# sparsemat/sprs

Measured on NVIDIA H100. Metric: csr_spmv_f64_gflops, higher is better.
Workload: dtype f64

## Files before the change

sprs_b200/csrc/common.cuh:

```cuda
#pragma once
#include <cuda_runtime.h>

#include <cstdint>
#include <cstdio>
#include <cstring>
#include <string>
#include <vector>

#include "../../include/sprs_b200.h"

constexpr int SPRS_E2E_MAX_CHUNKS = 8;
constexpr int SPRS_E2E_DEFAULT_CHUNKS = 8;

struct sprs_b200_ctx {
    int device = 0;
    int sm_count = 132;
    size_t l2_bytes = 0;
    cudaStream_t stream = nullptr;
    std::string last_error;
    uint64_t launches = 0;
    uint64_t pol_evict_first = 0, pol_evict_last = 0;
    void* h_stage = nullptr;
    size_t h_stage_bytes = 0;
    void* d_scratch[4] = {nullptr, nullptr, nullptr, nullptr};
    size_t d_scratch_bytes[4] = {0, 0, 0, 0};
    cudaStream_t side_stream = nullptr;
    cudaEvent_t ev_fork = nullptr, ev_join = nullptr;
    cudaStream_t copy_stream = nullptr;
    cudaEvent_t ev_chunk[SPRS_E2E_MAX_CHUNKS] = {};
    cudaEvent_t ev_copied = nullptr;
};

struct sprs_b200_csmat {
    sprs_b200_ctx* ctx = nullptr;
    int storage = SPRS_B200_CSR;
    uint64_t rows = 0, cols = 0, nnz = 0;
    uint64_t outer = 0, inner = 0;
    int indptr_bytes = 4;
    void* d_indptr = nullptr;
    uint32_t* d_indices = nullptr;
    double* d_data = nullptr;
    bool owns = true;
    bool pooled = false;
    uint32_t* d_tile_row = nullptr;
    void* d_tile_k = nullptr;
    double* d_carry = nullptr;
    uint64_t n_tiles = 0;
    uint32_t* d_hot_col = nullptr;
    uint32_t* d_hot_idx = nullptr;
    uint32_t n_hot = 0;
    mutable sprs_b200_csmat* csr_cache = nullptr;
    mutable std::vector<uint64_t> e2e_tiles, e2e_rows;
    mutable std::vector<uint64_t> push_tiles, push_rows;
};

#define SPRS_FAIL(ctx, code, ...)                                  \
    do {                                                           \
        char _buf[512];                                            \
        snprintf(_buf, sizeof(_buf), __VA_ARGS__);                 \
        sprs_b200_set_error((ctx), _buf);                          \
        return (code);                                             \
    } while (0)

#define SPRS_CUDA(ctx, expr)                                                              \
    do {                                                                                  \
        cudaError_t _e = (expr);                                                          \
        if (_e != cudaSuccess)                                                            \
            SPRS_FAIL((ctx), SPRS_B200_ERR_CUDA, "%s failed: %s (%s:%d)", #expr,          \
                      cudaGetErrorString(_e), __FILE__, __LINE__);                        \
    } while (0)

#define SPRS_TRY(expr)                      \
    do {                                    \
        int _s = (expr);                    \
        if (_s != SPRS_B200_OK) return _s;  \
    } while (0)

void sprs_b200_set_error(const sprs_b200_ctx* ctx, const char* msg);

static inline cudaStream_t pick_stream(sprs_b200_ctx*, void* stream) {
    return (cudaStream_t)stream;
}

int ctx_scratch(sprs_b200_ctx* ctx, int i, size_t bytes, void** out);
int ctx_stage(sprs_b200_ctx* ctx, size_t bytes, void** out);

constexpr int SPMV_MAX_TARGETS = 8;
struct SpmvTargets {
    double* p[SPMV_MAX_TARGETS];
    int n;
};

int spmv_prepare(sprs_b200_ctx* ctx, sprs_b200_csmat* m, cudaStream_t s, bool hot_set = true);
int spmv_tile_nnz();
int spmv_launch(sprs_b200_ctx* ctx, const sprs_b200_csmat* m, const double* d_x, double* d_y,
                int accumulate, cudaStream_t s);
int spmv_launch_targets(sprs_b200_ctx* ctx, const sprs_b200_csmat* m, const double* d_x,
                        const SpmvTargets& yt, int accumulate, cudaStream_t s);
int spmv_launch_tile_range(sprs_b200_ctx* ctx, const sprs_b200_csmat* m, const double* d_x,
                           double* d_y, int accumulate, uint64_t t0, uint64_t t1, cudaStream_t s);
int csmat_chunk_table(sprs_b200_ctx* ctx, const sprs_b200_csmat* m, uint64_t n_chunks, bool taper,
                      cudaStream_t s, std::vector<uint64_t>* tiles, std::vector<uint64_t>* rows);
int ctx_side_stream(sprs_b200_ctx* ctx);
// ... 24 lines not shown
```

sprs_b200/csrc/ptx.cuh:

```cuda
#pragma once
#include "common.cuh"

static __device__ __forceinline__ void fence_proxy_async() {
    asm volatile("fence.proxy.async.shared::cta;" ::: "memory");
}
static __device__ __forceinline__ uint64_t policy_evict_first() {
    uint64_t p;
    asm volatile("createpolicy.fractional.L2::evict_first.b64 %0, 1.0;" : "=l"(p));
    return p;
}
static __device__ __forceinline__ uint64_t policy_evict_last() {
    uint64_t p;
    asm volatile("createpolicy.fractional.L2::evict_last.b64 %0, 1.0;" : "=l"(p));
    return p;
}
static __device__ __forceinline__ double ldg_f64_hint(const double* p, uint64_t policy) {
    double v;
    asm("ld.global.nc.L2::cache_hint.f64 %0, [%1], %2;" : "=d"(v) : "l"(p), "l"(policy));
    return v;
}

static __device__ __forceinline__ uint32_t ldg_stream_u32(const uint32_t* p, uint64_t policy) {
    uint32_t v;
    asm("ld.global.nc.L1::no_allocate.L2::cache_hint.u32 %0, [%1], %2;"
        : "=r"(v) : "l"(p), "l"(policy));
    return v;
}
static __device__ __forceinline__ double ldg_stream_f64(const double* p, uint64_t policy) {
    double v;
    asm("ld.global.nc.L1::no_allocate.L2::cache_hint.f64 %0, [%1], %2;"
        : "=d"(v) : "l"(p), "l"(policy));
    return v;
}

static __device__ __forceinline__ void bulk_s2g(void* dst, const void* src_smem, uint32_t bytes) {
    asm volatile("cp.async.bulk.global.shared::cta.bulk_group [%0], [%1], %2;" ::"l"(dst),
                 "r"(smem_u32(src_smem)), "r"(bytes)
                 : "memory");
}
static __device__ __forceinline__ void bulk_commit_group() {
    asm volatile("cp.async.bulk.commit_group;" ::: "memory");
}
static __device__ __forceinline__ void bulk_wait_group_read0() {
    asm volatile("cp.async.bulk.wait_group.read 0;" ::: "memory");
}
static __device__ __forceinline__ void bulk_wait_group0() {
    asm volatile("cp.async.bulk.wait_group 0;" ::: "memory");
}
```

sprs_b200/csrc/spmv.cu:

```cuda

#include "common.cuh"
#include "ptx.cuh"
#include "scan.cuh"

#include <algorithm>
#include <cstdlib>

namespace {

constexpr int SPMV_STAGE_ROWS = 66;
constexpr uint32_t SPMV_ROW_COST = 16;

template <typename P>
__global__ void tile_cut_kernel(const P* __restrict__ indptr, uint32_t rows, uint64_t nnz,
                                uint64_t n_tiles, uint32_t w, uint32_t row_cost,
                                uint32_t* __restrict__ tile_row, P* __restrict__ tile_k) {
    const uint64_t t = blockIdx.x * (uint64_t)blockDim.x + threadIdx.x;
    if (t > n_tiles) return;
    if (t == n_tiles) {
        tile_row[t] = rows;
        tile_k[t] = (P)nnz;
        return;
    }
    const uint64_t d = t * (uint64_t)w;
    uint32_t lo = 0, hi = rows;
    while (lo < hi) {
        const uint32_t mid = lo + (hi - lo + 1) / 2;
        if ((uint64_t)indptr[mid] + (uint64_t)row_cost * mid <= d)
            lo = mid;
        else
            hi = mid - 1;
    }
    uint64_t k = d - (uint64_t)row_cost * lo;
    const uint64_t row_end = lo < rows ? (uint64_t)indptr[(size_t)lo + 1] : nnz;
    if (k > row_end) k = row_end;
    tile_row[t] = lo;
    tile_k[t] = (P)k;
}

struct RowSink {
    double* y;
    const SpmvTargets* yt;
    double* carry_slot;
    uint32_t r1;
    int accumulate;
    double* stage;
    uint32_t stage_off;
};
template <bool MULTI>
__device__ __forceinline__ void sink_row(const RowSink& k, uint64_t r, double sum) {
    if (r < k.r1) {
        const double v = k.accumulate ? __dadd_rn(k.y[r], sum) : sum;
        k.y[r] = v;
        if (MULTI) {
#pragma unroll
            if (k.stage) {
                k.stage[(uint32_t)r - k.stage_off] = v;
            } else {
#pragma unroll
                for (int q = 1; q < SPMV_MAX_TARGETS; ++q)
                    if (q < k.yt->n) k.yt->p[q][r] = v;
            }
        }
    } else {
        *k.carry_slot = sum;
    }
}

constexpr uint32_t HOT_TAG = 0x80000000u;
template <bool HOT>
__device__ __forceinline__ double gather_x(const double* __restrict__ x, const double* hot,
                                           uint32_t c, uint64_t polx) {
    if (HOT && (c & HOT_TAG)) return hot[c & ~HOT_TAG];
    return ldg_f64_hint(x + c, polx);
}

template <typename P, int G, int U, bool MULTI, bool HOT>
__device__ __forceinline__ void rows_direct(const RowSink& k, const P* __restrict__ indptr,
                                            const uint32_t* __restrict__ indices,
                                            const double* __restrict__ data,
                                            const double* __restrict__ x, const double* hot, P k0, P k1,
                                            uint32_t r0, uint32_t r_last, P b_first,
                                            uint64_t pol_stream, uint64_t polx, int lane) {
    constexpr int NG = 32 / G;
    constexpr unsigned FULL = 0xffffffffu;
    static_assert(G >= 4, "tiny rows have their own sweep: groups start at 4 lanes");
    const int gid = lane / G, gl = lane % G;
    P b = b_first;
    for (uint32_t rbase = r0;; rbase += 31) {
        if (rbase != r0) {
            const uint32_t rr = rbase + lane;
            b = (rr >= rbase && rr <= r_last + 1) ? indptr[rr] : (P)0;
        }
        const int nrows = (r_last - rbase + 1) < 31 ? (int)(r_last - rbase + 1) : 31;
        P ms = b, me = __shfl_down_sync(FULL, b, 1);
        ms = ms > k0 ? ms : k0;
        me = me < k1 ? me : k1;
        if (lane >= nrows || me < ms) me = ms;
        const bool tiny = lane < nrows && (me - ms) <= (P)(2 * U);
        if (__any_sync(FULL, tiny && me > ms)) {
            double acc = 0.0;
#pragma unroll
            for (int st = 0; st < 2; ++st) {
                const P q = ms + (P)(st * U);
                uint32_t c[U];
                double v[U], xv[U];
#pragma unroll
                for (int u = 0; u < U; ++u)
                    c[u] = (tiny && q + (P)u < me) ? ldg_stream_u32(indices + q + (P)u, pol_stream) : 0u;
#pragma unroll
                for (int u = 0; u < U; ++u)
                    v[u] = (tiny && q + (P)u < me) ? ldg_stream_f64(data + q + (P)u, pol_stream) : 0.0;
#pragma unroll
                for (int u = 0; u < U; ++u)
                    xv[u] = (tiny && q + (P)u < me) ? gather_x<HOT>(x, hot, c[u], polx) : 0.0;
#pragma unroll
                for (int u = 0; u < U; ++u)
                    if (tiny && q + (P)u < me) acc = __dadd_rn(acc, __dmul_rn(v[u], xv[u]));
                if (!__any_sync(FULL, tiny && q + (P)U < me)) break;
            }
            if (tiny) sink_row<MULTI>(k, (uint64_t)rbase + lane, acc);
        } else if (tiny) {
            sink_row<MULTI>(k, (uint64_t)rbase + lane, 0.0);
        }
        unsigned todo = __ballot_sync(FULL, lane < nrows && !tiny);
        while (todo) {
            int j = -1;
#pragma unroll
            for (int g = 0; g < NG; ++g) {
                if (todo) {
                    const int jj = __ffs(todo) - 1;
                    todo &= todo - 1;
                    if (gid == g) j = jj;
                }
            }
            const bool valid = j >= 0;
            const int js = valid ? j : 0;
            P s = __shfl_sync(FULL, b, js);
            P e = __shfl_sync(FULL, b, js + 1);
            s = s > k0 ? s : k0;
            e = e < k1 ? e : k1;
            if (!valid || e < s) e = s;
            const bool is_long = (G < 32) && (e - s) > (P)(4 * G * U);
            double acc = 0.0;
            for (P q = s + gl; q < (is_long ? s : e); q += (P)(G * U)) {
                uint32_t c[U];
                double v[U], xv[U];
#pragma unroll
                for (int u = 0; u < U; ++u)
                    c[u] = q + (P)(u * G) < e ? ldg_stream_u32(indices + q + (P)(u * G), pol_stream) : 0u;
#pragma unroll
                for (int u = 0; u < U; ++u)
                    v[u] = q + (P)(u * G) < e ? ldg_stream_f64(data + q + (P)(u * G), pol_stream) : 0.0;
#pragma unroll
                for (int u = 0; u < U; ++u)
                    xv[u] = q + (P)(u * G) < e ? gather_x<HOT>(x, hot, c[u], polx) : 0.0;
#pragma unroll
                for (int u = 0; u < U; ++u)
                    if (q + (P)(u * G) < e) acc = __dadd_rn(acc, __dmul_rn(v[u], xv[u]));
            }
#pragma unroll
            for (int o = G / 2; o > 0; o >>= 1) acc = __dadd_rn(acc, __shfl_xor_sync(FULL, acc, o));
            if (gl == 0 && valid && !is_long) sink_row<MULTI>(k, (uint64_t)rbase + j, acc);
            if (G < 32) {
                unsigned pending = __ballot_sync(FULL, gl == 0 && is_long);
                while (pending) {
                    const int src = __ffs(pending) - 1;
                    pending &= pending - 1;
                    const P qs = __shfl_sync(FULL, s, src), qe = __shfl_sync(FULL, e, src);
                    const int jj = __shfl_sync(FULL, j, src);
                    double a2 = 0.0;
                    for (P q = qs + lane; q < qe; q += (P)(32 * U)) {
                        uint32_t c[U];
                        double v[U], xv[U];
#pragma unroll
                        for (int u = 0; u < U; ++u)
                            c[u] = q + (P)(u * 32) < qe ? ldg_stream_u32(indices + q + (P)(u * 32), pol_stream) : 0u;
#pragma unroll
                        for (int u = 0; u < U; ++u)
                            v[u] = q + (P)(u * 32) < qe ? ldg_stream_f64(data + q + (P)(u * 32), pol_stream) : 0.0;
#pragma unroll
                        for (int u = 0; u < U; ++u)
                            xv[u] = q + (P)(u * 32) < qe ? gather_x<HOT>(x, hot, c[u], polx) : 0.0;
#pragma unroll
                        for (int u = 0; u < U; ++u)
                            if (q + (P)(u * 32) < qe) a2 = __dadd_rn(a2, __dmul_rn(v[u], xv[u]));
                    }
#pragma unroll
                    for (int o = 16; o > 0; o >>= 1) a2 = __dadd_rn(a2, __shfl_xor_sync(FULL, a2, o));
                    if (lane == 0) sink_row<MULTI>(k, (uint64_t)rbase + jj, a2);
                }
            }
        }
        if (r_last - rbase < 31) break;
    }
}

template <typename P, int NWARPS, int MINB, int U, bool MULTI, bool HOT>
__global__ void __launch_bounds__(NWARPS * 32, MINB)
    spmv_rows_kernel(const P* __restrict__ indptr, const uint32_t* __restrict__ indices,
                     const double* __restrict__ data, const uint32_t* __restrict__ tile_row,
                     const P* __restrict__ tile_k, const double* __restrict__ x,
                     const __grid_constant__ SpmvTargets yt,
                     double* __restrict__ carry, uint64_t nnz, uint32_t rows, uint32_t t_begin,
                     uint32_t t_end , int accumulate,
                     uint64_t pol_stream , uint64_t polx ,
                     int stage_rows ,
                     const uint32_t* __restrict__ hot_col ,
                     uint32_t n_hot) {
    const int lane = threadIdx.x & 31, warp = threadIdx.x >> 5;
    extern __shared__ __align__(16) double hot_x[];
    if constexpr (HOT) {
        for (uint32_t q = threadIdx.x; q < n_hot; q += NWARPS * 32)
            hot_x[q] = ldg_f64_hint(x + hot_col[q], polx);
        __syncthreads();
    }
    const uint32_t GW = gridDim.x * NWARPS;
    RowSink sink;
    sink.y = yt.p[0];
    sink.yt = &yt;
    sink.accumulate = accumulate;
    sink.stage = nullptr;
    sink.stage_off = 0;
    double* my_stage = nullptr;
    if constexpr (MULTI) {
        __shared__ __align__(16) double stage_all[NWARPS * SPMV_STAGE_ROWS];
        my_stage = stage_all + warp * SPMV_STAGE_ROWS;
    }
    const uint32_t par = MULTI ? (uint32_t)(((uintptr_t)yt.p[1] >> 3) & 1) : 0u;
    uint32_t t = t_begin + blockIdx.x * NWARPS + warp;
    if (t >= t_end) return;
    uint32_t r0 = tile_row[t], r1 = tile_row[t + 1];
    P k0 = tile_k[t], k1 = tile_k[t + 1];
    P b_first = (uint64_t)r0 + lane <= (r1 < rows ? (uint64_t)r1 + 1 : (uint64_t)r1)
                    ? indptr[(size_t)r0 + lane] : (P)0;
    for (;;) {
        const uint32_t tn = t + GW;
        uint32_t r0n = 0, r1n = 0;
        P k0n = 0, k1n = 0;
        if (tn < t_end) {
            r0n = tile_row[tn];
            r1n = tile_row[tn + 1];
            k0n = tile_k[tn];
            k1n = tile_k[tn + 1];
        }
        sink.carry_slot = carry + t;
        sink.r1 = r1;
        if (MULTI && stage_rows) {
            const uint32_t base = (r0 + par) & ~1u;
            const bool fits = r1 > r0 && (r1 + par - base) <= (uint32_t)SPMV_STAGE_ROWS;
            sink.stage = fits ? my_stage : nullptr;
            sink.stage_off = base - par;
            if (fits) {
                if (lane == 0) bulk_wait_group_read0();
                __syncwarp();
            }
        }
        const uint32_t r_last = r1 < rows ? r1 : r1 - 1;
        const uint64_t cnt = k1 - k0, nr = (uint64_t)(r_last - r0) + 1;
#define SPMV_ROWS(G)                                                                            \
    rows_direct<P, G, U, MULTI, HOT>(sink, indptr, indices, data, x, hot_x, k0, k1, r0, r_last,   \
                                     b_first, pol_stream, polx, lane)
        if (cnt <= 24 * nr)
            SPMV_ROWS(4);
        else if (cnt <= 48 * nr)
            SPMV_ROWS(8);
        else if (cnt <= 96 * nr)
            SPMV_ROWS(16);
        else
            SPMV_ROWS(32);
#undef SPMV_ROWS
        if (MULTI && sink.stage) {
            fence_proxy_async();
            __syncwarp();
            if (lane == 0) {
                uint32_t lo = r0, hi = r1;
                if ((lo + par) & 1u) {
                    const double v = my_stage[lo - sink.stage_off];
                    for (int q = 1; q < yt.n; ++q) yt.p[q][lo] = v;
                    ++lo;
                }
                if ((hi - lo) & 1u) {
                    --hi;
                    const double v = my_stage[hi - sink.stage_off];
                    for (int q = 1; q < yt.n; ++q) yt.p[q][hi] = v;
                }
                if (hi > lo) {
                    for (int q = 1; q < yt.n; ++q)
                        bulk_s2g(yt.p[q] + lo, my_stage + (lo - sink.stage_off), (hi - lo) * 8u);
                    bulk_commit_group();
                }
            }
            sink.stage = nullptr;
        }
        if (tn >= t_end) break;
        const P b_next = (uint64_t)r0n + lane <= (r1n < rows ? (uint64_t)r1n + 1 : (uint64_t)r1n)
                             ? indptr[(size_t)r0n + lane] : (P)0;
        t = tn;
        r0 = r0n;
        r1 = r1n;
        k0 = k0n;
        k1 = k1n;
        b_first = b_next;
    }
    if (MULTI && stage_rows && lane == 0) bulk_wait_group0();
}

__global__ void spmv_fixup_kernel(const uint32_t* __restrict__ tile_row,
                                  const double* __restrict__ carry, SpmvTargets yt,
                                  uint64_t n_tiles) {
    const uint64_t t = blockIdx.x * (uint64_t)blockDim.x + threadIdx.x;
    if (t + 1 >= n_tiles) return;
    const uint32_t row = tile_row[t + 1];
    if (t > 0 && tile_row[t] == row) return;
    uint64_t lo = t + 1, hi = n_tiles - 1;
    for (uint64_t step = 1; lo + step < hi; step <<= 1) {
        if (tile_row[lo + step + 1] > row) {
            hi = lo + step;
            break;
        }
        lo += step;
    }
    while (lo < hi) {
        const uint64_t mid = lo + (hi - lo) / 2;
        if (tile_row[mid + 1] > row)
            hi = mid;
        else
            lo = mid + 1;
    }
    double sum = carry[t];
#pragma unroll 8
    for (uint64_t u = t + 1; u < lo; ++u) sum = __dadd_rn(sum, carry[u]);
    const double v = __dadd_rn(yt.p[0][row], sum);
#pragma unroll
    for (int q = 0; q < SPMV_MAX_TARGETS; ++q)
        if (q < yt.n) yt.p[q][row] = v;
}

__device__ __forceinline__ void apply_carries_ending_in(const uint32_t* __restrict__ tile_row,
                                                        const double* carry, double* y,
                                                        uint64_t u) {
    const uint32_t row = tile_row[u];
    if (tile_row[u + 1] == row) return;
    uint64_t hi = u, lo = 1;
    for (uint64_t step = 1; step < hi; step <<= 1) {
        if (tile_row[hi - step] < row) {
            lo = hi - step + 1;
            break;
        }
        hi -= step;
    }
    while (lo < hi) {
        const uint64_t mid = lo + (hi - lo) / 2;
        if (tile_row[mid] >= row)
            hi = mid;
        else
            lo = mid + 1;
    }
    double sum = __ldcg(carry + lo - 1);
    for (uint64_t v = lo; v < u; ++v) sum = __dadd_rn(sum, __ldcg(carry + v));
    y[row] = __dadd_rn(__ldcg(y + row), sum);
}

__global__ void spmv_fixup_range_kernel(const uint32_t* __restrict__ tile_row, const double* carry,
                                        double* y, uint64_t u_lo, uint64_t u_hi) {
    const uint64_t u = u_lo + blockIdx.x * (uint64_t)blockDim.x + threadIdx.x;
    if (u >= 1 && u < u_hi) apply_carries_ending_in(tile_row, carry, y, u);
}

struct SpmvVariant {
    int wt, row_cost;
};
SpmvVariant spmv_variant() {
    static SpmvVariant v = [] {
        SpmvVariant d{1024, (int)SPMV_ROW_COST};
        if (const char* e = getenv("SPRS_B200_SPMV_VARIANT")) {
            int a, rc = (int)SPMV_ROW_COST;
            const int got = sscanf(e, "%d,%d", &a, &rc);
            if (got >= 1 && a >= 64 && rc >= 0) d = SpmvVariant{a, rc};
        }
        return d;
    }();
    return v;
}

constexpr int SPMV_NWARPS = 8, SPMV_CTAS_PER_SM = 5, SPMV_LOADS_IN_FLIGHT = 4;

constexpr int SPMV_HOT_NWARPS = 32, SPMV_HOT_CTAS_PER_SM = 1;
constexpr uint32_t SPMV_HOT_SLOTS = 24576;
constexpr uint32_t SPMV_HOT_MAX_SLOTS = 26624;
constexpr uint64_t SPMV_HOT_MIN_NNZ = 1ull << 25;
constexpr double SPMV_HOT_MIN_SHARE = 0.10;

struct SpmvHot {
    uint32_t k;
    bool forced;
};
SpmvHot spmv_hot() {
    static SpmvHot h = [] {
        SpmvHot d{SPMV_HOT_SLOTS, false};
        const char* e = getenv("SPRS_B200_SPMV_HOT");
        if (e && strcmp(e, "auto") != 0) {
            const long k = atol(e);
            d = SpmvHot{(uint32_t)(k < 0 ? 0 : k > (long)SPMV_HOT_MAX_SLOTS ? SPMV_HOT_MAX_SLOTS : k), true};
        }
        return d;
    }();
    return h;
}

template <typename P, bool MULTI, bool HOT>
auto* spmv_kernel() {
    constexpr int U = SPMV_LOADS_IN_FLIGHT;
    if constexpr (HOT)
        return spmv_rows_kernel<P, SPMV_HOT_NWARPS, SPMV_HOT_CTAS_PER_SM, U, MULTI, true>;
    else
        return spmv_rows_kernel<P, SPMV_NWARPS, SPMV_CTAS_PER_SM, U, MULTI, false>;
}

template <typename P>
int launch_variant(sprs_b200_ctx* ctx, const sprs_b200_csmat* m, const double* d_x,
                   const SpmvTargets& yt, int accumulate, uint64_t t0, uint64_t t1,
                   cudaStream_t s) {
    if (m->n_tiles >= 0xffffffffull)
        SPRS_FAIL(ctx, SPRS_B200_ERR_UNSUPPORTED, "spmv: more than 2^32 tiles");
    const bool multi = yt.n > 1, hot = m->n_hot > 0;
    auto kern = hot ? (multi ? spmv_kernel<P, true, true>() : spmv_kernel<P, false, true>())
                    : (multi ? spmv_kernel<P, true, false>() : spmv_kernel<P, false, false>());
    const int nwarps = hot ? SPMV_HOT_NWARPS : SPMV_NWARPS;
    const int ctas = hot ? SPMV_HOT_CTAS_PER_SM : SPMV_CTAS_PER_SM;
    static bool configured_flags[64][4] = {};
    bool& configured = configured_flags[ctx->device & 63][(multi ? 1 : 0) + (hot ? 2 : 0)];
    if (!configured) {
        int carve;
        if (hot) {
            const int dyn = (int)(spmv_hot().k * sizeof(double));
            const int per_cta = dyn + (multi ? nwarps * SPMV_STAGE_ROWS * 8 : 0) + 1024;
            SPRS_CUDA(ctx, cudaFuncSetAttribute(kern, cudaFuncAttributeMaxDynamicSharedMemorySize, dyn));
            carve = (int)((100ull * ctas * per_cta + 228 * 1024 - 1) / (228 * 1024));
        } else {
            carve = multi ? 15 : 0;
            if (const char* e = getenv("SPRS_B200_SPMV_CARVEOUT")) carve = atoi(e);
        }
        SPRS_CUDA(ctx, cudaFuncSetAttribute(kern, cudaFuncAttributePreferredSharedMemoryCarveout,
                                            carve));
        configured = true;
    }
    int stage_rows = 0;
    if (multi) {
        stage_rows = yt.n > 2 ? SPMV_STAGE_ROWS : 0;
        if (const char* e = getenv("SPRS_B200_SPMV_PEER_STORES")) {
            if (e[0] == 'd') stage_rows = 0;
            if (e[0] == 't') stage_rows = SPMV_STAGE_ROWS;
        }
        for (int q = 2; q < yt.n; ++q)
            if ((((uintptr_t)yt.p[q] ^ (uintptr_t)yt.p[1]) >> 3) & 1) stage_rows = 0;
    }
    uint64_t grid = (uint64_t)ctx->sm_count * ctas;
    const uint64_t need = (t1 - t0 + nwarps - 1) / nwarps;
    if (grid > need) grid = need;
    const size_t smem = hot ? m->n_hot * sizeof(double) : 0;
    kern<<<(unsigned)grid, nwarps * 32, smem, s>>>((const P*)m->d_indptr,
                                                   hot ? m->d_hot_idx : m->d_indices,
                                                   m->d_data, m->d_tile_row, (const P*)m->d_tile_k, d_x, yt,
                                                   m->d_carry,
                                                   m->nnz, (uint32_t)m->rows, (uint32_t)t0,
                                                   (uint32_t)t1, accumulate, ctx->pol_evict_first,
                                                   ctx->pol_evict_last, stage_rows, m->d_hot_col,
                                                   m->n_hot);
    return SPRS_B200_OK;
}

__device__ __forceinline__ void add_aggregated(uint32_t* counts, uint32_t key, unsigned active) {
    const unsigned peers = __match_any_sync(active, key);
    if ((int)(threadIdx.x & 31) == __ffs(peers) - 1) atomicAdd(counts + key, (uint32_t)__popc(peers));
}

__global__ void hot_count_kernel(const uint32_t* __restrict__ indices, uint64_t nnz,
                                 uint32_t* __restrict__ counts) {
    const uint64_t stride = (uint64_t)gridDim.x * blockDim.x;
    for (uint64_t base = blockIdx.x * (uint64_t)blockDim.x + (threadIdx.x & ~31u); base < nnz;
         base += stride) {
        const uint64_t i = base + (threadIdx.x & 31);
        const bool valid = i < nnz;
        const unsigned active = __ballot_sync(0xffffffffu, valid);
        if (valid) add_aggregated(counts, indices[i], active);
    }
}

__global__ void hot_count_hist_kernel(const uint32_t* __restrict__ counts, uint32_t cols,
                                      uint32_t hi, uint32_t* __restrict__ hist) {
    const uint64_t stride = (uint64_t)gridDim.x * blockDim.x;
    for (uint64_t base = blockIdx.x * (uint64_t)blockDim.x + (threadIdx.x & ~31u); base < cols;
         base += stride) {
        const uint64_t i = base + (threadIdx.x & 31);
        const uint32_t c = i < cols ? counts[i] : 0u;
        const bool take = c > 0 && (hi == ~0u || (c >> 16) == hi);
        const unsigned active = __ballot_sync(0xffffffffu, take);
        if (take) add_aggregated(hist, hi == ~0u ? c >> 16 : c & 0xffffu, active);
    }
}

__global__ void hot_flag_kernel(const uint32_t* __restrict__ counts, uint32_t cols, uint32_t thr,
                                const uint32_t* __restrict__ tie_rank, uint32_t ties,
                                uint8_t* __restrict__ flag) {
    const uint64_t i = blockIdx.x * (uint64_t)blockDim.x + threadIdx.x;
    if (i >= cols) return;
    const uint32_t c = counts[i];
    flag[i] = tie_rank ? (c > thr || (c == thr && tie_rank[i] < ties)) : c == thr;
}

__global__ void hot_map_kernel(uint32_t* __restrict__ counts_map, uint32_t cols,
                               const uint8_t* __restrict__ sel, const uint32_t* __restrict__ slot,
                               uint32_t* __restrict__ hot_col, unsigned long long* hot_nnz) {
    const uint64_t i = blockIdx.x * (uint64_t)blockDim.x + threadIdx.x;
    if (i >= cols) return;
    if (sel[i]) {
        const uint32_t q = slot[i];
        atomicAdd(hot_nnz, (unsigned long long)counts_map[i]);
        hot_col[q] = (uint32_t)i;
        counts_map[i] = HOT_TAG | q;
    } else {
        counts_map[i] = (uint32_t)i;
    }
}

__global__ void hot_tag_kernel(const uint32_t* __restrict__ indices, uint64_t nnz,
                               const uint32_t* __restrict__ map, uint32_t* __restrict__ tagged) {
    const uint64_t stride = (uint64_t)gridDim.x * blockDim.x;
    for (uint64_t i = blockIdx.x * (uint64_t)blockDim.x + threadIdx.x; i < nnz; i += stride)
        tagged[i] = map[indices[i]];
}

int spmv_prepare_hot(sprs_b200_ctx* ctx, sprs_b200_csmat* m, cudaStream_t s) {
    const SpmvHot cfg = spmv_hot();
    if (cfg.k == 0 || m->nnz == 0 || m->cols == 0 || m->cols >= HOT_TAG) return SPRS_B200_OK;
    if (!cfg.forced && m->nnz < SPMV_HOT_MIN_NNZ) return SPRS_B200_OK;
    const uint32_t cols = (uint32_t)m->cols;
    uint32_t *counts = nullptr, *hist = nullptr, *slot = nullptr, *hot_col = nullptr,
             *hot_idx = nullptr;
    uint8_t* flag = nullptr;
    unsigned long long* d_hot_nnz = nullptr;
    const unsigned grid_nnz =
        (unsigned)std::min<uint64_t>((m->nnz + 255) / 256, (uint64_t)ctx->sm_count * 16);
    const unsigned grid_cols = (unsigned)((cols + 255) / 256);
    auto build = [&]() -> int {
        if (cudaMalloc((void**)&counts, cols * sizeof(uint32_t)) != cudaSuccess ||
            cudaMalloc((void**)&hist, 65536 * sizeof(uint32_t)) != cudaSuccess ||
            cudaMalloc((void**)&flag, cols) != cudaSuccess ||
            cudaMalloc((void**)&slot, (cols + 1ull) * sizeof(uint32_t)) != cudaSuccess ||
            cudaMalloc((void**)&d_hot_nnz, sizeof(unsigned long long)) != cudaSuccess)
            return SPRS_B200_OK;
        SPRS_CUDA(ctx, cudaMemsetAsync(counts, 0, cols * sizeof(uint32_t), s));
        SPRS_CUDA(ctx, cudaMemsetAsync(hist, 0, 65536 * sizeof(uint32_t), s));
        SPRS_CUDA(ctx, cudaMemsetAsync(d_hot_nnz, 0, sizeof(unsigned long long), s));
        hot_count_kernel<<<grid_nnz, 256, 0, s>>>(m->d_indices, m->nnz, counts);
        hot_count_hist_kernel<<<grid_cols, 256, 0, s>>>(counts, cols, ~0u, hist);
        ctx->launches += 2;
        std::vector<uint32_t> h(65536);
        SPRS_CUDA(ctx, cudaMemcpyAsync(h.data(), hist, 65536 * sizeof(uint32_t),
                                       cudaMemcpyDeviceToHost, s));
        SPRS_CUDA(ctx, cudaStreamSynchronize(s));
        uint64_t above = 0, referenced = 0;
        for (uint32_t b = 0; b < 65536; ++b) referenced += h[b];
        uint32_t k = cfg.k, thr = 1, ties = 0xffffffffu;
        if (referenced > k) {
            uint32_t bhi = 65535;
            while (above + h[bhi] < k) above += h[bhi--];
            SPRS_CUDA(ctx, cudaMemsetAsync(hist, 0, 65536 * sizeof(uint32_t), s));
            hot_count_hist_kernel<<<grid_cols, 256, 0, s>>>(counts, cols, bhi, hist);
            ctx->launches += 1;
            SPRS_CUDA(ctx, cudaMemcpyAsync(h.data(), hist, 65536 * sizeof(uint32_t),
                                           cudaMemcpyDeviceToHost, s));
            SPRS_CUDA(ctx, cudaStreamSynchronize(s));
            uint32_t blo = 65535;
            while (above + h[blo] < k) above += h[blo--];
            thr = (bhi << 16) | blo;
            ties = k - (uint32_t)above;
        } else {
            k = (uint32_t)referenced;
        }
        hot_flag_kernel<<<grid_cols, 256, 0, s>>>(counts, cols, thr, nullptr, 0, flag);
        ctx->launches += 1;
        SPRS_TRY((device_exclusive_scan<uint8_t, uint32_t>(ctx, flag, cols, slot, s)));
        hot_flag_kernel<<<grid_cols, 256, 0, s>>>(counts, cols, thr, slot, ties, flag);
        ctx->launches += 1;
        SPRS_TRY((device_exclusive_scan<uint8_t, uint32_t>(ctx, flag, cols, slot, s)));
        if (cudaMalloc((void**)&hot_col, k * sizeof(uint32_t)) != cudaSuccess) return SPRS_B200_OK;
        hot_map_kernel<<<grid_cols, 256, 0, s>>>(counts, cols, flag, slot, hot_col, d_hot_nnz);
        ctx->launches += 1;
        unsigned long long hot_nnz = 0;
        SPRS_CUDA(ctx, cudaMemcpyAsync(&hot_nnz, d_hot_nnz, sizeof(hot_nnz), cudaMemcpyDeviceToHost, s));
        SPRS_CUDA(ctx, cudaStreamSynchronize(s));
        if (!cfg.forced && (double)hot_nnz < SPMV_HOT_MIN_SHARE * (double)m->nnz) return SPRS_B200_OK;
        if (cudaMalloc((void**)&hot_idx, m->nnz * sizeof(uint32_t) + 16) != cudaSuccess)
            return SPRS_B200_OK;
        hot_tag_kernel<<<grid_nnz, 256, 0, s>>>(m->d_indices, m->nnz, counts, hot_idx);
        ctx->launches += 1;
        SPRS_CUDA(ctx, cudaStreamSynchronize(s));
        SPRS_CUDA(ctx, cudaGetLastError());
        m->d_hot_col = hot_col;
        m->d_hot_idx = hot_idx;
        m->n_hot = k;
        return SPRS_B200_OK;
    };
    const int st = build();
    if (m->n_hot == 0) {
        cudaGetLastError();
        if (hot_col) cudaFree(hot_col);
        if (hot_idx) cudaFree(hot_idx);
    }
    if (counts) cudaFree(counts);
    if (hist) cudaFree(hist);
    if (flag) cudaFree(flag);
    if (slot) cudaFree(slot);
    if (d_hot_nnz) cudaFree(d_hot_nnz);
    return st;
}

int check_spmv_args(sprs_b200_ctx* ctx, const sprs_b200_csmat* m) {
    if (m->storage != SPRS_B200_CSR)
        SPRS_FAIL(ctx, SPRS_B200_ERR_STORAGE, "Storage mismatch: spmv needs a CSR mirror");
    if (!m->d_tile_row) SPRS_FAIL(ctx, SPRS_B200_ERR_ARGUMENT, "csmat has no SpMV partition");
    return SPRS_B200_OK;
}

}

int spmv_tile_nnz() { return spmv_variant().wt; }

int spmv_prepare(sprs_b200_ctx* ctx, sprs_b200_csmat* m, cudaStream_t s, bool hot_set) {
    if (m->storage != SPRS_B200_CSR) return SPRS_B200_OK;
    const uint32_t w = (uint32_t)spmv_tile_nnz();
    const uint32_t row_cost = (uint32_t)spmv_variant().row_cost;
    const uint64_t total = m->nnz + (uint64_t)row_cost * m->rows;
    m->n_tiles = total == 0 ? 1 : (total + w - 1) / w;
    SPRS_CUDA(ctx, cudaMalloc((void**)&m->d_tile_row, (m->n_tiles + 1) * sizeof(uint32_t)));
    SPRS_CUDA(ctx, cudaMalloc((void**)&m->d_tile_k, (m->n_tiles + 1) * (size_t)m->indptr_bytes));
    SPRS_CUDA(ctx, cudaMalloc((void**)&m->d_carry, m->n_tiles * sizeof(double)));
    const uint64_t n = m->n_tiles + 1;
    const unsigned grid = (unsigned)((n + 255) / 256);
    if (m->indptr_bytes == 4)
        tile_cut_kernel<uint32_t><<<grid, 256, 0, s>>>((const uint32_t*)m->d_indptr, (uint32_t)m->rows,
                                                       m->nnz, m->n_tiles, w, row_cost, m->d_tile_row,
                                                       (uint32_t*)m->d_tile_k);
    else
        tile_cut_kernel<uint64_t><<<grid, 256, 0, s>>>((const uint64_t*)m->d_indptr, (uint32_t)m->rows,
                                                       m->nnz, m->n_tiles, w, row_cost, m->d_tile_row,
                                                       (uint64_t*)m->d_tile_k);
    ctx->launches += 1;
    SPRS_CUDA(ctx, cudaGetLastError());
    if (hot_set) SPRS_TRY(spmv_prepare_hot(ctx, m, s));
    return SPRS_B200_OK;
}

int spmv_launch_targets(sprs_b200_ctx* ctx, const sprs_b200_csmat* m, const double* d_x,
                        const SpmvTargets& yt, int accumulate, cudaStream_t s) {
    SPRS_TRY(check_spmv_args(ctx, m));
    if (m->rows == 0) return SPRS_B200_OK;
    if (m->indptr_bytes == 4)
        SPRS_TRY(launch_variant<uint32_t>(ctx, m, d_x, yt, accumulate, 0, m->n_tiles, s));
    else
        SPRS_TRY(launch_variant<uint64_t>(ctx, m, d_x, yt, accumulate, 0, m->n_tiles, s));
    ctx->launches += 1;
    if (m->n_tiles > 1) {
        const unsigned fgrid = (unsigned)((m->n_tiles - 1 + 255) / 256);
        spmv_fixup_kernel<<<fgrid, 256, 0, s>>>(m->d_tile_row, m->d_carry, yt, m->n_tiles);
        ctx->launches += 1;
// ... 34 lines not shown
```

Measured before the change: 226.9.

## Split hot x cache across CTA pairs via clusters and distributed shared memory

Extends the shared-memory cache of frequently referenced x entries by launching the hot SpMV kernel as 2-CTA clusters. A small set of the hottest columns is duplicated in each CTA, and a larger set is split between the pair, with remote entries read through DSMEM (mapa + ld.shared::cluster). This roughly doubles effective cached x capacity to cut L2/HBM gathers, at the cost of cluster barriers at kernel start and exit, slower remote shared loads, and more preprocessing kernels and host syncs.

Result: faster. 230.7 (median of 6 runs) (+1.7%).

```diff
diff --git a/sprs_b200/csrc/common.cuh b/sprs_b200/csrc/common.cuh
--- a/sprs_b200/csrc/common.cuh
+++ b/sprs_b200/csrc/common.cuh
@@ -49,6 +49,7 @@
     uint32_t* d_hot_col = nullptr;
     uint32_t* d_hot_idx = nullptr;
     uint32_t n_hot = 0;
+    uint32_t n_hot_split = 0;
     mutable sprs_b200_csmat* csr_cache = nullptr;
     mutable std::vector<uint64_t> e2e_tiles, e2e_rows;
     mutable std::vector<uint64_t> push_tiles, push_rows;
diff --git a/sprs_b200/csrc/ptx.cuh b/sprs_b200/csrc/ptx.cuh
--- a/sprs_b200/csrc/ptx.cuh
+++ b/sprs_b200/csrc/ptx.cuh
@@ -33,6 +33,25 @@
     return v;
 }
 
+static __device__ __forceinline__ uint32_t cluster_ctarank() {
+    uint32_t r;
+    asm volatile("mov.u32 %0, %%cluster_ctarank;" : "=r"(r));
+    return r;
+}
+static __device__ __forceinline__ void cluster_arrive_release() {
+    asm volatile("barrier.cluster.arrive.release;" ::: "memory");
+}
+static __device__ __forceinline__ void cluster_wait_acquire() {
+    asm volatile("barrier.cluster.wait.acquire;" ::: "memory");
+}
+static __device__ __forceinline__ double ld_dsmem_f64(const double* p, uint32_t rank) {
+    uint32_t a;
+    double v;
+    asm volatile("mapa.shared::cluster.u32 %0, %1, %2;" : "=r"(a) : "r"(smem_u32(p)), "r"(rank));
+    asm volatile("ld.shared::cluster.f64 %0, [%1];" : "=d"(v) : "r"(a));
+    return v;
+}
+
 static __device__ __forceinline__ void bulk_s2g(void* dst, const void* src_smem, uint32_t bytes) {
     asm volatile("cp.async.bulk.global.shared::cta.bulk_group [%0], [%1], %2;" ::"l"(dst),
                  "r"(smem_u32(src_smem)), "r"(bytes)
diff --git a/sprs_b200/csrc/spmv.cu b/sprs_b200/csrc/spmv.cu
--- a/sprs_b200/csrc/spmv.cu
+++ b/sprs_b200/csrc/spmv.cu
@@ -67,21 +67,36 @@
     }
 }
 
-constexpr uint32_t HOT_TAG = 0x80000000u;
-template <bool HOT>
+constexpr uint32_t HOT_TAG = 0x80000000u, HOT_SPLIT = 0x40000000u, HOT_OWNER_SHIFT = 29,
+                   HOT_SLOT = 0x1fffffffu;
+enum { HOT_OFF = 0, HOT_CTA = 1, HOT_CLUSTER = 2 };
+#ifdef __NVCC__
+#define SPMV_HOT_CLUSTERS 1
+#else
+#define SPMV_HOT_CLUSTERS 0
+#endif
+template <int HOT>
 __device__ __forceinline__ double gather_x(const double* __restrict__ x, const double* hot,
-                                           uint32_t c, uint64_t polx) {
-    if (HOT && (c & HOT_TAG)) return hot[c & ~HOT_TAG];
+                                           uint32_t c, uint64_t polx, uint32_t rank) {
+    if (HOT != HOT_OFF && (c & HOT_TAG)) {
+        const double* p = hot + (c & HOT_SLOT);
+#if SPMV_HOT_CLUSTERS
+        if (HOT == HOT_CLUSTER && (c & HOT_SPLIT) && ((c >> HOT_OWNER_SHIFT) & 1u) != rank)
+            return ld_dsmem_f64(p, rank ^ 1u);
+#endif
+        return *p;
+    }
     return ldg_f64_hint(x + c, polx);
 }
 
-template <typename P, int G, int U, bool MULTI, bool HOT>
+template <typename P, int G, int U, bool MULTI, int HOT>
 __device__ __forceinline__ void rows_direct(const RowSink& k, const P* __restrict__ indptr,
                                             const uint32_t* __restrict__ indices,
                                             const double* __restrict__ data,
                                             const double* __restrict__ x, const double* hot, P k0, P k1,
                                             uint32_t r0, uint32_t r_last, P b_first,
-                                            uint64_t pol_stream, uint64_t polx, int lane) {
+                                            uint64_t pol_stream, uint64_t polx, int lane,
+                                            uint32_t rank) {
     constexpr int NG = 32 / G;
     constexpr unsigned FULL = 0xffffffffu;
     static_assert(G >= 4, "tiny rows have their own sweep: groups start at 4 lanes");
@@ -113,7 +128,7 @@
                     v[u] = (tiny && q + (P)u < me) ? ldg_stream_f64(data + q + (P)u, pol_stream) : 0.0;
 #pragma unroll
                 for (int u = 0; u < U; ++u)
-                    xv[u] = (tiny && q + (P)u < me) ? gather_x<HOT>(x, hot, c[u], polx) : 0.0;
+                    xv[u] = (tiny && q + (P)u < me) ? gather_x<HOT>(x, hot, c[u], polx, rank) : 0.0;
 #pragma unroll
                 for (int u = 0; u < U; ++u)
                     if (tiny && q + (P)u < me) acc = __dadd_rn(acc, __dmul_rn(v[u], xv[u]));
@@ -154,7 +169,7 @@
                     v[u] = q + (P)(u * G) < e ? ldg_stream_f64(data + q + (P)(u * G), pol_stream) : 0.0;
 #pragma unroll
                 for (int u = 0; u < U; ++u)
-                    xv[u] = q + (P)(u * G) < e ? gather_x<HOT>(x, hot, c[u], polx) : 0.0;
+                    xv[u] = q + (P)(u * G) < e ? gather_x<HOT>(x, hot, c[u], polx, rank) : 0.0;
 #pragma unroll
                 for (int u = 0; u < U; ++u)
                     if (q + (P)(u * G) < e) acc = __dadd_rn(acc, __dmul_rn(v[u], xv[u]));
@@ -181,7 +196,7 @@
                             v[u] = q + (P)(u * 32) < qe ? ldg_stream_f64(data + q + (P)(u * 32), pol_stream) : 0.0;
 #pragma unroll
                         for (int u = 0; u < U; ++u)
-                            xv[u] = q + (P)(u * 32) < qe ? gather_x<HOT>(x, hot, c[u], polx) : 0.0;
+                            xv[u] = q + (P)(u * 32) < qe ? gather_x<HOT>(x, hot, c[u], polx, rank) : 0.0;
 #pragma unroll
                         for (int u = 0; u < U; ++u)
                             if (q + (P)(u * 32) < qe) a2 = __dadd_rn(a2, __dmul_rn(v[u], xv[u]));
@@ -196,7 +211,17 @@
     }
 }
 
-template <typename P, int NWARPS, int MINB, int U, bool MULTI, bool HOT>
+template <int HOT>
+__device__ __forceinline__ void hot_cluster_exit() {
+#if SPMV_HOT_CLUSTERS
+    if constexpr (HOT == HOT_CLUSTER) {
+        cluster_arrive_release();
+        cluster_wait_acquire();
+    }
+#endif
+}
+
+template <typename P, int NWARPS, int MINB, int U, bool MULTI, int HOT>
 __global__ void __launch_bounds__(NWARPS * 32, MINB)
     spmv_rows_kernel(const P* __restrict__ indptr, const uint32_t* __restrict__ indices,
                      const double* __restrict__ data, const uint32_t* __restrict__ tile_row,
@@ -207,14 +232,25 @@
                      uint64_t pol_stream , uint64_t polx ,
                      int stage_rows ,
                      const uint32_t* __restrict__ hot_col ,
-                     uint32_t n_hot) {
+                     uint32_t n_hot, uint32_t n_dup ) {
     const int lane = threadIdx.x & 31, warp = threadIdx.x >> 5;
     extern __shared__ __align__(16) double hot_x[];
-    if constexpr (HOT) {
+    uint32_t rank = 0;
+    if constexpr (HOT == HOT_CTA) {
         for (uint32_t q = threadIdx.x; q < n_hot; q += NWARPS * 32)
             hot_x[q] = ldg_f64_hint(x + hot_col[q], polx);
         __syncthreads();
     }
+#if SPMV_HOT_CLUSTERS
+    if constexpr (HOT == HOT_CLUSTER) {
+        rank = cluster_ctarank();
+        const uint32_t n_mine = n_dup + (n_hot - n_dup + 1 - rank) / 2;
+        for (uint32_t q = threadIdx.x; q < n_mine; q += NWARPS * 32)
+            hot_x[q] = ldg_f64_hint(x + hot_col[q < n_dup ? q : n_dup + 2 * (q - n_dup) + rank], polx);
+        cluster_arrive_release();
+        cluster_wait_acquire();
+    }
+#endif
     const uint32_t GW = gridDim.x * NWARPS;
     RowSink sink;
     sink.y = yt.p[0];
@@ -229,7 +265,10 @@
     }
     const uint32_t par = MULTI ? (uint32_t)(((uintptr_t)yt.p[1] >> 3) & 1) : 0u;
     uint32_t t = t_begin + blockIdx.x * NWARPS + warp;
-    if (t >= t_end) return;
+    if (t >= t_end) {
+        hot_cluster_exit<HOT>();
+        return;
+    }
     uint32_t r0 = tile_row[t], r1 = tile_row[t + 1];
     P k0 = tile_k[t], k1 = tile_k[t + 1];
     P b_first = (uint64_t)r0 + lane <= (r1 < rows ? (uint64_t)r1 + 1 : (uint64_t)r1)
@@ -260,7 +299,7 @@
         const uint64_t cnt = k1 - k0, nr = (uint64_t)(r_last - r0) + 1;
 #define SPMV_ROWS(G)                                                                            \
     rows_direct<P, G, U, MULTI, HOT>(sink, indptr, indices, data, x, hot_x, k0, k1, r0, r_last,   \
-                                     b_first, pol_stream, polx, lane)
+                                     b_first, pol_stream, polx, lane, rank)
         if (cnt <= 24 * nr)
             SPMV_ROWS(4);
         else if (cnt <= 48 * nr)
@@ -304,6 +343,7 @@
         b_first = b_next;
     }
     if (MULTI && stage_rows && lane == 0) bulk_wait_group0();
+    hot_cluster_exit<HOT>();
 }
 
 __global__ void spmv_fixup_kernel(const uint32_t* __restrict__ tile_row,
@@ -387,35 +427,114 @@
 constexpr int SPMV_NWARPS = 8, SPMV_CTAS_PER_SM = 5, SPMV_LOADS_IN_FLIGHT = 4;
 
 constexpr int SPMV_HOT_NWARPS = 32, SPMV_HOT_CTAS_PER_SM = 1;
-constexpr uint32_t SPMV_HOT_SLOTS = 24576;
 constexpr uint32_t SPMV_HOT_MAX_SLOTS = 26624;
+constexpr uint32_t SPMV_HOT_AUTO_DUP = 4096, SPMV_HOT_AUTO_SPLIT = 16384;
 constexpr uint64_t SPMV_HOT_MIN_NNZ = 1ull << 25;
 constexpr double SPMV_HOT_MIN_SHARE = 0.10;
 
 struct SpmvHot {
-    uint32_t k;
+    uint32_t dup, split;
     bool forced;
+    uint32_t per_cta() const { return dup + split; }
 };
 SpmvHot spmv_hot() {
     static SpmvHot h = [] {
-        SpmvHot d{SPMV_HOT_SLOTS, false};
+        SpmvHot d{SPMV_HOT_AUTO_DUP, SPMV_HOT_AUTO_SPLIT, false};
         const char* e = getenv("SPRS_B200_SPMV_HOT");
         if (e && strcmp(e, "auto") != 0) {
-            const long k = atol(e);
-            d = SpmvHot{(uint32_t)(k < 0 ? 0 : k > (long)SPMV_HOT_MAX_SLOTS ? SPMV_HOT_MAX_SLOTS : k), true};
+            const char* plus = strchr(e, '+');
+            long a = atol(e), b = plus ? atol(plus + 1) : 0;
+            a = a < 0 ? 0 : a > (long)SPMV_HOT_MAX_SLOTS ? SPMV_HOT_MAX_SLOTS : a;
+            b = b < 0 ? 0 : b > (long)SPMV_HOT_MAX_SLOTS - a ? SPMV_HOT_MAX_SLOTS - a : b;
+            d = SpmvHot{(uint32_t)a, (uint32_t)b, true};
         }
         return d;
     }();
     return h;
 }
 
-template <typename P, bool MULTI, bool HOT>
-auto* spmv_kernel() {
-    constexpr int U = SPMV_LOADS_IN_FLIGHT;
-    if constexpr (HOT)
-        return spmv_rows_kernel<P, SPMV_HOT_NWARPS, SPMV_HOT_CTAS_PER_SM, U, MULTI, true>;
-    else
-        return spmv_rows_kernel<P, SPMV_NWARPS, SPMV_CTAS_PER_SM, U, MULTI, false>;
+template <typename P>
+using SpmvKernel = decltype(&spmv_rows_kernel<P, SPMV_NWARPS, SPMV_CTAS_PER_SM,
+                                              SPMV_LOADS_IN_FLIGHT, false, HOT_OFF>);
+template <typename P>
+SpmvKernel<P> spmv_kernel(bool multi, int hot) {
+    constexpr int U = SPMV_LOADS_IN_FLIGHT, HW = SPMV_HOT_NWARPS, HB = SPMV_HOT_CTAS_PER_SM;
+    switch (hot) {
+        case HOT_CTA:
+            return multi ? spmv_rows_kernel<P, HW, HB, U, true, HOT_CTA>
+                         : spmv_rows_kernel<P, HW, HB, U, false, HOT_CTA>;
+        case HOT_CLUSTER:
+            return multi ? spmv_rows_kernel<P, HW, HB, U, true, HOT_CLUSTER>
+                         : spmv_rows_kernel<P, HW, HB, U, false, HOT_CLUSTER>;
+        default:
+            return multi ? spmv_rows_kernel<P, SPMV_NWARPS, SPMV_CTAS_PER_SM, U, true, HOT_OFF>
+                         : spmv_rows_kernel<P, SPMV_NWARPS, SPMV_CTAS_PER_SM, U, false, HOT_OFF>;
+    }
+}
+
+template <typename P>
+int configure_spmv_kernel(sprs_b200_ctx* ctx, bool multi, int hot) {
+    static bool configured_flags[64][6] = {};
+    bool& configured = configured_flags[ctx->device & 63][(multi ? 1 : 0) + 2 * hot];
+    if (configured) return SPRS_B200_OK;
+    auto kern = spmv_kernel<P>(multi, hot);
+    int carve;
+    if (hot != HOT_OFF) {
+        const int dyn = (int)(spmv_hot().per_cta() * sizeof(double));
+        const int per_cta = dyn + (multi ? SPMV_HOT_NWARPS * SPMV_STAGE_ROWS * 8 : 0) + 1024;
+        SPRS_CUDA(ctx, cudaFuncSetAttribute(kern, cudaFuncAttributeMaxDynamicSharedMemorySize, dyn));
+        carve = (int)((100ull * SPMV_HOT_CTAS_PER_SM * per_cta + 228 * 1024 - 1) / (228 * 1024));
+    } else {
+        carve = multi ? 15 : 0;
+        if (const char* e = getenv("SPRS_B200_SPMV_CARVEOUT")) carve = atoi(e);
+    }
+    SPRS_CUDA(ctx, cudaFuncSetAttribute(kern, cudaFuncAttributePreferredSharedMemoryCarveout, carve));
+    configured = true;
+    return SPRS_B200_OK;
+}
+
+#if SPMV_HOT_CLUSTERS
+cudaLaunchConfig_t hot_cluster_config(unsigned grid, size_t smem, cudaStream_t s,
+                                      cudaLaunchAttribute* attr) {
+    cudaLaunchConfig_t c = {};
+    c.gridDim = dim3(grid);
+    c.blockDim = dim3(SPMV_HOT_NWARPS * 32);
+    c.dynamicSmemBytes = smem;
+    c.stream = s;
+    attr->id = cudaLaunchAttributeClusterDimension;
+    attr->val.clusterDim.x = 2;
+    attr->val.clusterDim.y = 1;
+    attr->val.clusterDim.z = 1;
+    c.attrs = attr;
+    c.numAttrs = 1;
+    return c;
+}
+#endif
+
+template <typename P>
+bool hot_cluster_fits(sprs_b200_ctx* ctx) {
+#if !SPMV_HOT_CLUSTERS
+    (void)ctx;
+    return false;
+#else
+    static int fits[64] = {};
+    int& f = fits[ctx->device & 63];
+    if (f == 0) {
+        f = 2;
+        if (configure_spmv_kernel<P>(ctx, false, HOT_CLUSTER) == SPRS_B200_OK) {
+            cudaLaunchAttribute attr;
+            const unsigned grid = (unsigned)ctx->sm_count & ~1u;
+            const cudaLaunchConfig_t c =
+                hot_cluster_config(grid, spmv_hot().per_cta() * sizeof(double), nullptr, &attr);
+            int n = 0;
+            if (cudaOccupancyMaxActiveClusters(&n, spmv_kernel<P>(false, HOT_CLUSTER), &c) == cudaSuccess &&
+                2u * (unsigned)n >= grid && grid > 0)
+                f = 1;
+        }
+        cudaGetLastError();
+    }
+    return f == 1;
+#endif
 }
 
 template <typename P>
@@ -424,28 +543,12 @@
                    cudaStream_t s) {
     if (m->n_tiles >= 0xffffffffull)
         SPRS_FAIL(ctx, SPRS_B200_ERR_UNSUPPORTED, "spmv: more than 2^32 tiles");
-    const bool multi = yt.n > 1, hot = m->n_hot > 0;
-    auto kern = hot ? (multi ? spmv_kernel<P, true, true>() : spmv_kernel<P, false, true>())
-                    : (multi ? spmv_kernel<P, true, false>() : spmv_kernel<P, false, false>());
-    const int nwarps = hot ? SPMV_HOT_NWARPS : SPMV_NWARPS;
-    const int ctas = hot ? SPMV_HOT_CTAS_PER_SM : SPMV_CTAS_PER_SM;
-    static bool configured_flags[64][4] = {};
-    bool& configured = configured_flags[ctx->device & 63][(multi ? 1 : 0) + (hot ? 2 : 0)];
-    if (!configured) {
-        int carve;
-        if (hot) {
-            const int dyn = (int)(spmv_hot().k * sizeof(double));
-            const int per_cta = dyn + (multi ? nwarps * SPMV_STAGE_ROWS * 8 : 0) + 1024;
-            SPRS_CUDA(ctx, cudaFuncSetAttribute(kern, cudaFuncAttributeMaxDynamicSharedMemorySize, dyn));
-            carve = (int)((100ull * ctas * per_cta + 228 * 1024 - 1) / (228 * 1024));
-        } else {
-            carve = multi ? 15 : 0;
-            if (const char* e = getenv("SPRS_B200_SPMV_CARVEOUT")) carve = atoi(e);
-        }
-        SPRS_CUDA(ctx, cudaFuncSetAttribute(kern, cudaFuncAttributePreferredSharedMemoryCarveout,
-                                            carve));
-        configured = true;
-    }
+    const bool multi = yt.n > 1;
+    const int hot = m->n_hot == 0 ? HOT_OFF : m->n_hot_split ? HOT_CLUSTER : HOT_CTA;
+    auto kern = spmv_kernel<P>(multi, hot);
+    const int nwarps = hot != HOT_OFF ? SPMV_HOT_NWARPS : SPMV_NWARPS;
+    const int ctas = hot != HOT_OFF ? SPMV_HOT_CTAS_PER_SM : SPMV_CTAS_PER_SM;
+    SPRS_TRY(configure_spmv_kernel<P>(ctx, multi, hot));
     int stage_rows = 0;
     if (multi) {
         stage_rows = yt.n > 2 ? SPMV_STAGE_ROWS : 0;
@@ -459,15 +562,31 @@
     uint64_t grid = (uint64_t)ctx->sm_count * ctas;
     const uint64_t need = (t1 - t0 + nwarps - 1) / nwarps;
     if (grid > need) grid = need;
-    const size_t smem = hot ? m->n_hot * sizeof(double) : 0;
-    kern<<<(unsigned)grid, nwarps * 32, smem, s>>>((const P*)m->d_indptr,
-                                                   hot ? m->d_hot_idx : m->d_indices,
+    const uint32_t n_dup = m->n_hot - m->n_hot_split;
+    const size_t smem = hot == HOT_CLUSTER ? (n_dup + (m->n_hot_split + 1) / 2) * sizeof(double)
+                                           : m->n_hot * sizeof(double);
+    const uint32_t* idx = hot != HOT_OFF ? m->d_hot_idx : m->d_indices;
+#if SPMV_HOT_CLUSTERS
+    if (hot == HOT_CLUSTER) {
+        grid = (grid + 1) & ~1ull;
+        cudaLaunchAttribute attr;
+        const cudaLaunchConfig_t c = hot_cluster_config((unsigned)grid, smem, s, &attr);
+        SPRS_CUDA(ctx, cudaLaunchKernelEx(&c, kern, (const P*)m->d_indptr, idx, (const double*)m->d_data,
+                                          (const uint32_t*)m->d_tile_row, (const P*)m->d_tile_k, d_x, yt,
+                                          m->d_carry, m->nnz, (uint32_t)m->rows, (uint32_t)t0,
+                                          (uint32_t)t1, accumulate, ctx->pol_evict_first,
+                                          ctx->pol_evict_last, stage_rows,
+                                          (const uint32_t*)m->d_hot_col, m->n_hot, n_dup));
+        return SPRS_B200_OK;
+    }
+#endif
+    kern<<<(unsigned)grid, nwarps * 32, smem, s>>>((const P*)m->d_indptr, idx,
                                                    m->d_data, m->d_tile_row, (const P*)m->d_tile_k, d_x, yt,
                                                    m->d_carry,
                                                    m->nnz, (uint32_t)m->rows, (uint32_t)t0,
                                                    (uint32_t)t1, accumulate, ctx->pol_evict_first,
                                                    ctx->pol_evict_last, stage_rows, m->d_hot_col,
-                                                   m->n_hot);
+                                                   m->n_hot, n_dup);
     return SPRS_B200_OK;
 }
 
@@ -512,6 +631,8 @@
 
 __global__ void hot_map_kernel(uint32_t* __restrict__ counts_map, uint32_t cols,
                                const uint8_t* __restrict__ sel, const uint32_t* __restrict__ slot,
+                               const uint8_t* __restrict__ split,
+                               const uint32_t* __restrict__ split_slot, uint32_t n_dup,
                                uint32_t* __restrict__ hot_col, unsigned long long* hot_nnz) {
     const uint64_t i = blockIdx.x * (uint64_t)blockDim.x + threadIdx.x;
     if (i >= cols) return;
@@ -520,9 +641,19 @@
         atomicAdd(hot_nnz, (unsigned long long)counts_map[i]);
         hot_col[q] = (uint32_t)i;
         counts_map[i] = HOT_TAG | q;
+    } else if (split && split[i]) {
+        const uint32_t j = split_slot[i];
+        atomicAdd(hot_nnz, (unsigned long long)counts_map[i]);
+        hot_col[n_dup + j] = (uint32_t)i;
+        counts_map[i] = HOT_TAG | HOT_SPLIT | (j & 1u) << HOT_OWNER_SHIFT | (n_dup + (j >> 1));
     } else {
         counts_map[i] = (uint32_t)i;
     }
+}
+
+__global__ void hot_minus_kernel(uint8_t* __restrict__ a, const uint8_t* __restrict__ b, uint32_t cols) {
+    const uint64_t i = blockIdx.x * (uint64_t)blockDim.x + threadIdx.x;
+    if (i < cols) a[i] = a[i] && !b[i];
 }
 
 __global__ void hot_tag_kernel(const uint32_t* __restrict__ indices, uint64_t nnz,
@@ -534,12 +665,16 @@
 
 int spmv_prepare_hot(sprs_b200_ctx* ctx, sprs_b200_csmat* m, cudaStream_t s) {
     const SpmvHot cfg = spmv_hot();
-    if (cfg.k == 0 || m->nnz == 0 || m->cols == 0 || m->cols >= HOT_TAG) return SPRS_B200_OK;
+    if (cfg.per_cta() == 0 || m->nnz == 0 || m->cols == 0 || m->cols >= HOT_TAG) return SPRS_B200_OK;
     if (!cfg.forced && m->nnz < SPMV_HOT_MIN_NNZ) return SPRS_B200_OK;
+    const bool cluster = cfg.split > 0 && (m->indptr_bytes == 4 ? hot_cluster_fits<uint32_t>(ctx)
+                                                                : hot_cluster_fits<uint64_t>(ctx));
+    const uint32_t want_dup = cluster ? cfg.dup : cfg.per_cta();
+    const uint32_t want_all = cluster ? cfg.dup + 2 * cfg.split : cfg.per_cta();
     const uint32_t cols = (uint32_t)m->cols;
-    uint32_t *counts = nullptr, *hist = nullptr, *slot = nullptr, *hot_col = nullptr,
-             *hot_idx = nullptr;
-    uint8_t* flag = nullptr;
+    uint32_t *counts = nullptr, *hist = nullptr, *slot = nullptr, *slot2 = nullptr,
+             *hot_col = nullptr, *hot_idx = nullptr;
+    uint8_t *flag = nullptr, *flag2 = nullptr;
     unsigned long long* d_hot_nnz = nullptr;
     const unsigned grid_nnz =
         (unsigned)std::min<uint64_t>((m->nnz + 255) / 256, (uint64_t)ctx->sm_count * 16);
@@ -551,43 +686,64 @@
             cudaMalloc((void**)&slot, (cols + 1ull) * sizeof(uint32_t)) != cudaSuccess ||
             cudaMalloc((void**)&d_hot_nnz, sizeof(unsigned long long)) != cudaSuccess)
             return SPRS_B200_OK;
+        if (want_all > want_dup &&
+            (cudaMalloc((void**)&flag2, cols) != cudaSuccess ||
+             cudaMalloc((void**)&slot2, (cols + 1ull) * sizeof(uint32_t)) != cudaSuccess))
+            return SPRS_B200_OK;
         SPRS_CUDA(ctx, cudaMemsetAsync(counts, 0, cols * sizeof(uint32_t), s));
         SPRS_CUDA(ctx, cudaMemsetAsync(hist, 0, 65536 * sizeof(uint32_t), s));
         SPRS_CUDA(ctx, cudaMemsetAsync(d_hot_nnz, 0, sizeof(unsigned long long), s));
         hot_count_kernel<<<grid_nnz, 256, 0, s>>>(m->d_indices, m->nnz, counts);
         hot_count_hist_kernel<<<grid_cols, 256, 0, s>>>(counts, cols, ~0u, hist);
         ctx->launches += 2;
-        std::vector<uint32_t> h(65536);
-        SPRS_CUDA(ctx, cudaMemcpyAsync(h.data(), hist, 65536 * sizeof(uint32_t),
+        std::vector<uint32_t> h_hi(65536), h(65536);
+        SPRS_CUDA(ctx, cudaMemcpyAsync(h_hi.data(), hist, 65536 * sizeof(uint32_t),
                                        cudaMemcpyDeviceToHost, s));
         SPRS_CUDA(ctx, cudaStreamSynchronize(s));
-        uint64_t above = 0, referenced = 0;
-        for (uint32_t b = 0; b < 65536; ++b) referenced += h[b];
-        uint32_t k = cfg.k, thr = 1, ties = 0xffffffffu;
-        if (referenced > k) {
-            uint32_t bhi = 65535;
-            while (above + h[bhi] < k) above += h[bhi--];
-            SPRS_CUDA(ctx, cudaMemsetAsync(hist, 0, 65536 * sizeof(uint32_t), s));
-            hot_count_hist_kernel<<<grid_cols, 256, 0, s>>>(counts, cols, bhi, hist);
+        uint64_t referenced = 0;
+        for (uint32_t b = 0; b < 65536; ++b) referenced += h_hi[b];
+        auto select_top = [&](uint32_t k, uint8_t* f, uint32_t* sl, uint32_t& got) -> int {
+            uint32_t thr = 1, ties = 0xffffffffu;
+            if (referenced > k) {
+                uint64_t above = 0;
+                uint32_t bhi = 65535;
+                while (above + h_hi[bhi] < k) above += h_hi[bhi--];
+                SPRS_CUDA(ctx, cudaMemsetAsync(hist, 0, 65536 * sizeof(uint32_t), s));
+                hot_count_hist_kernel<<<grid_cols, 256, 0, s>>>(counts, cols, bhi, hist);
+                ctx->launches += 1;
+                SPRS_CUDA(ctx, cudaMemcpyAsync(h.data(), hist, 65536 * sizeof(uint32_t),
+                                               cudaMemcpyDeviceToHost, s));
+                SPRS_CUDA(ctx, cudaStreamSynchronize(s));
+                uint32_t blo = 65535;
+                while (above + h[blo] < k) above += h[blo--];
+                thr = (bhi << 16) | blo;
+                ties = k - (uint32_t)above;
+                got = k;
+            } else {
+                got = (uint32_t)referenced;
+            }
+            hot_flag_kernel<<<grid_cols, 256, 0, s>>>(counts, cols, thr, nullptr, 0, f);
             ctx->launches += 1;
-            SPRS_CUDA(ctx, cudaMemcpyAsync(h.data(), hist, 65536 * sizeof(uint32_t),
-                                           cudaMemcpyDeviceToHost, s));
-            SPRS_CUDA(ctx, cudaStreamSynchronize(s));
-            uint32_t blo = 65535;
-            while (above + h[blo] < k) above += h[blo--];
-            thr = (bhi << 16) | blo;
-            ties = k - (uint32_t)above;
+            SPRS_TRY((device_exclusive_scan<uint8_t, uint32_t>(ctx, f, cols, sl, s)));
+            hot_flag_kernel<<<grid_cols, 256, 0, s>>>(counts, cols, thr, sl, ties, f);
+            ctx->launches += 1;
+            SPRS_TRY((device_exclusive_scan<uint8_t, uint32_t>(ctx, f, cols, sl, s)));
+            return SPRS_B200_OK;
+        };
+        uint32_t n_all = 0, n_dup = 0;
+        if (flag2) {
+            SPRS_TRY(select_top(want_all, flag2, slot2, n_all));
+            SPRS_TRY(select_top(want_dup, flag, slot, n_dup));
+            hot_minus_kernel<<<grid_cols, 256, 0, s>>>(flag2, flag, cols);
+            ctx->launches += 1;
+            SPRS_TRY((device_exclusive_scan<uint8_t, uint32_t>(ctx, flag2, cols, slot2, s)));
         } else {
-            k = (uint32_t)referenced;
-        }
-        hot_flag_kernel<<<grid_cols, 256, 0, s>>>(counts, cols, thr, nullptr, 0, flag);
-        ctx->launches += 1;
-        SPRS_TRY((device_exclusive_scan<uint8_t, uint32_t>(ctx, flag, cols, slot, s)));
-        hot_flag_kernel<<<grid_cols, 256, 0, s>>>(counts, cols, thr, slot, ties, flag);
-        ctx->launches += 1;
-        SPRS_TRY((device_exclusive_scan<uint8_t, uint32_t>(ctx, flag, cols, slot, s)));
-        if (cudaMalloc((void**)&hot_col, k * sizeof(uint32_t)) != cudaSuccess) return SPRS_B200_OK;
-        hot_map_kernel<<<grid_cols, 256, 0, s>>>(counts, cols, flag, slot, hot_col, d_hot_nnz);
+            SPRS_TRY(select_top(want_dup, flag, slot, n_dup));
+            n_all = n_dup;
+        }
+        if (cudaMalloc((void**)&hot_col, n_all * sizeof(uint32_t)) != cudaSuccess) return SPRS_B200_OK;
+        hot_map_kernel<<<grid_cols, 256, 0, s>>>(counts, cols, flag, slot, flag2, slot2, n_dup,
+                                                 hot_col, d_hot_nnz);
         ctx->launches += 1;
         unsigned long long hot_nnz = 0;
         SPRS_CUDA(ctx, cudaMemcpyAsync(&hot_nnz, d_hot_nnz, sizeof(hot_nnz), cudaMemcpyDeviceToHost, s));
@@ -601,7 +757,8 @@
         SPRS_CUDA(ctx, cudaGetLastError());
         m->d_hot_col = hot_col;
         m->d_hot_idx = hot_idx;
-        m->n_hot = k;
+        m->n_hot = n_all;
+        m->n_hot_split = n_all - n_dup;
         return SPRS_B200_OK;
     };
     const int st = build();
@@ -614,6 +771,8 @@
     if (hist) cudaFree(hist);
     if (flag) cudaFree(flag);
     if (slot) cudaFree(slot);
+    if (flag2) cudaFree(flag2);
+    if (slot2) cudaFree(slot2);
     if (d_hot_nnz) cudaFree(d_hot_nnz);
     return st;
 }
```
